# jsnchon/acai-omr

Measured on AMD Instinct MI355X. Metric: LMX tokens/sec (greedy decode, KV cache), higher is better.
Workload: dtype bf16; 1 GPU; vitomr_greedy_decode batch 8/GPU of 512x2048 images (4096 patches), decode steps 6..136; batch_per_gpu=8, memory_len=4096, decoder=12 x d1024 h16 mlp4096, V=227, hipgraph=True, split_merge=in-launch

## Files before the change

### acai_omr_amd/_lib.py

```python
import ctypes
import os
import subprocess
from ctypes import POINTER, Structure, c_char_p, c_double, c_float, c_int, c_int32, c_int64, c_uint32, c_void_p, c_size_t

CSRC = os.path.join(os.path.dirname(os.path.abspath(__file__)), "csrc")
LIB_PATH = os.environ.get("ACAI_OMR_LIB") or os.path.join(CSRC, "libacai_omr_hip.so")
SOURCES = ["gemm.hip", "gemm_tile.hip", "gemm_ring.hip", "gemm_pp.hip", "elementwise.hip", "attn.hip", "attn_varlen.hip", "attn_probs.hip", "confidence.hip", "attn_fwd64.hip", "attn_fwd64w.hip", "attn_bwd.hip", "attn_bwd64w.hip", "attn_bwd1p.hip", "train.hip", "grpo.hip", "seqdist.hip", "seqalign.hip", "grammar.hip", "decode.hip", "decode_gemv.hip", "decode_attn.hip", "decode_select.hip", "decode_prefill.hip", "resize.hip", "augment.hip", "page.hip", "deskew.hip", "flatten.hip", "rectify.hip", "ingest.hip", "prune.hip", "assess.hip"]

ACAI_F32, ACAI_BF16, ACAI_FP8_E4M3 = 0, 1, 2
GEMM_GELU, GEMM_ROUND_BF16 = 1, 2
(GEMM_K_REG, GEMM_K_GLDS, GEMM_K_GLDS3, GEMM_K_PERS, GEMM_K_256, GEMM_K_PERS256, GEMM_K_PP, GEMM_K_TN_GLDS, GEMM_K_TN_RING,
 GEMM_K_TN_PP) = range(10)
GEMM_KERNEL_NAMES = ("gemm_nt_kernel", "gemm_nt_glds_kernel", "gemm_nt_glds3_kernel", "gemm_nt_pers_kernel", "gemm_nt_256_kernel",
                     "gemm_nt_pers256_kernel", "gemm_nt_pp_kernel", "gemm_tn_glds_kernel", "gemm_tn_ring_kernel", "gemm_tn_pp_kernel")
GEMM_PP_OBF, GEMM_PP_GELU, GEMM_PP_AUX1, GEMM_PP_AUX2, GEMM_PP_RES, GEMM_PP_SCALE, GEMM_PP_DEFER, GEMM_PP_AUX3, GEMM_PP_AUX4 = 1, 2, 4, 8, 16, 32, 64, 128, 256
DEC_CROSS_FP8 = 256


class AcaiDecLayer(Structure):
    _fields_ = [(n, c_void_p) for n in (
        "self_in_w", "self_in_b", "self_out_w", "self_out_b", "cross_q_w", "cross_q_b", "cross_out_w", "cross_out_b",
        "lin1_w", "lin1_b", "lin2_w", "lin2_b", "n1_w", "n1_b", "n2_w", "n2_b", "n3_w", "n3_b",
        "k_self", "v_self", "k_cross", "v_cross", "k_cross_scale", "v_cross_scale")]

# ... 177 lines not shown
    "acai_page_warp": (c_int, [c_void_p, c_int, c_int, c_int, c_int, POINTER(c_int64), c_float, c_void_p, c_int, c_int, c_int, c_void_p]),
    "acai_page_ingest": (c_int, [c_void_p, c_int, c_int, c_int, c_int, c_int64, c_int64, c_int64, c_int, c_void_p, c_int, c_void_p]),
    "acai_page_col_profile": (c_int, [c_void_p, c_int, c_int, c_int, c_int, c_float, c_void_p, c_void_p, c_void_p, c_int64, c_void_p]),
    "acai_page_box_ink": (c_int, [c_void_p, c_int, c_int, c_int, c_int, c_float, c_void_p, c_int, c_void_p, c_void_p]),
    "acai_page_runs": (c_int, [c_void_p, c_int, c_int, c_int, c_int, c_float, c_void_p, c_void_p, c_int64, c_void_p]),
    "acai_page_sharpness": (c_int, [c_void_p, c_int, c_int, c_int, c_int, c_void_p, c_void_p]),
    "acai_patch_ink": (c_int, [c_void_p, c_int, c_int, c_int, c_int64, c_float, c_void_p, c_void_p]),
    "acai_patch_keep": (c_int, [c_void_p, c_void_p, c_int, c_int, c_int, c_int, c_void_p, c_void_p, c_void_p]),
    "acai_patch_compact": (c_int, [c_void_p, c_int, c_int, c_int64, c_void_p, c_void_p, c_void_p, c_int, c_int, c_void_p, c_void_p, c_void_p, c_void_p]),
    "acai_attn_map_expand": (c_int, [c_void_p, c_void_p, c_void_p, c_void_p, c_void_p, c_void_p, c_void_p, c_void_p, c_int, c_int, c_int, c_void_p]),
    "acai_gather_rows": (c_int, [c_void_p, c_void_p, c_void_p, c_void_p, c_int, c_int, c_void_p]),
    "acai_attn_varlen_fwd": (c_int, [c_void_p, c_int, c_void_p, c_int, c_void_p, c_int, c_void_p, c_int, c_void_p, c_void_p,
                                     c_int, c_int, c_int, c_int, c_int, c_int, c_void_p, c_int, c_float, c_uint32, c_int, c_void_p]),
    "acai_attn_probs_mean": (c_int, [c_void_p, c_int, c_void_p, c_int, c_void_p, c_void_p, c_int, c_int, c_int, c_int, c_int, c_int, c_void_p, c_int,
                                     c_void_p, c_void_p, c_void_p, c_int, c_void_p]),
    "acai_attn_map_locate": (c_int, [c_void_p, c_void_p, c_void_p, c_void_p, POINTER(c_int32), c_int, c_int, c_void_p, c_void_p, c_void_p]),
    "acai_token_confidence": (c_int, [c_void_p, c_void_p, c_int, c_int, c_int, c_float, c_void_p, c_void_p, c_void_p, c_void_p, c_void_p, c_void_p]),
    "acai_attn_map_weighted_sum": (c_int, [c_void_p, c_void_p, c_void_p, c_void_p, c_void_p, c_int, c_int, c_int, c_int64, c_void_p, c_void_p,
                                           c_void_p]),
    "acai_attn_varlen_bwd": (c_int, [c_void_p, c_int, c_void_p, c_int, c_void_p, c_int, c_void_p, c_int, c_void_p, c_int, c_void_p, c_int,
                                     c_void_p, c_int, c_void_p, c_int, c_void_p, c_void_p, c_void_p, c_void_p, c_int, c_int, c_int, c_int, c_int,
                                     c_int, c_int, c_int, c_float, c_uint32, c_int, c_void_p]),
    "acai_attn_varlen_bwd_ws": (c_int, [c_void_p, c_int, c_void_p, c_int, c_void_p, c_int, c_void_p, c_int, c_void_p, c_int, c_void_p, c_int,
                                        c_void_p, c_int, c_void_p, c_int, c_void_p, c_void_p, c_void_p, c_void_p, c_int, c_int, c_int, c_int, c_int,
                                        c_int, c_int, c_int, c_int, c_float, c_uint32, c_int, c_void_p, c_size_t, c_void_p]),
    "acai_attn_varlen_bwd_workspace_bytes": (c_size_t, [c_int, c_int, c_int, c_int, c_int, c_int, c_int, c_int, c_int, c_float, c_int]),
    "acai_attn_plan": (c_int, [POINTER(AcaiAttnQuery), POINTER(AcaiAttnLaunch), POINTER(c_int), POINTER(c_int)]),
    "acai_attn_last_plan": (c_int, [POINTER(AcaiAttnLaunch), POINTER(c_int)]),
    "acai_attn_set_override": (c_int, [c_int, c_int]),
    "acai_attn_get_override": (c_int, [c_int, POINTER(c_int)]),
    "acai_dropout_add": (c_int, [c_void_p, c_void_p, c_void_p, c_int, c_int, c_float, c_uint32, c_int, c_int, c_void_p]),
    "acai_layernorm_bwd": (c_int, [c_void_p, c_void_p, c_void_p, c_float, c_void_p, c_void_p, c_void_p, c_void_p, c_void_p, c_void_p, c_int, c_int, c_void_p]),
    "acai_gelu_fwd": (c_int, [c_void_p, c_void_p, c_int64, c_int, c_void_p]),
    "acai_gelu_bwd": (c_int, [c_void_p, c_void_p, c_void_p, c_int64, c_int, c_void_p]),
    "acai_adamw_step": (c_int, [c_void_p, c_void_p, c_void_p, c_void_p, c_int, c_int, c_float, c_void_p]),
    "acai_grad_norm": (c_int, [c_void_p, c_void_p, c_void_p, c_void_p, c_int, c_int, c_int, c_float, c_float, c_void_p, c_void_p, c_void_p, c_void_p]),
    "acai_adamw_step_clipped": (c_int, [c_void_p, c_void_p, c_void_p, c_void_p, c_int, c_int, c_float, c_void_p, c_int, c_void_p, c_void_p]),
    "acai_cast_weights": (c_int, [c_void_p, c_int, c_int, c_void_p]),
    "acai_gemm_dw": (c_int, [c_void_p, c_int, c_void_p, c_int, c_void_p, c_int, c_void_p, c_int, c_int, c_int, c_int, c_void_p]),
    "acai_colsum": (c_int, [c_void_p, c_int, c_void_p, c_int, c_int, c_int, c_void_p]),
    "acai_scatter_add_rows": (c_int, [c_void_p, c_void_p, c_void_p, c_int, c_int, c_int, c_void_p]),
    "acai_mae_loss": (c_int, [c_void_p, c_void_p, c_void_p, c_float, c_void_p, c_void_p, c_int, c_int, c_void_p]),
    "acai_ce_loss": (c_int, [c_void_p, c_int, c_void_p, c_int, c_float, c_float, c_void_p, c_void_p, c_int, c_int, c_void_p]),
    "acai_grpo_objective_fwd": (c_int, [c_void_p, c_int, c_void_p, c_int, c_void_p, c_int, c_void_p, c_void_p, c_int, c_int, c_int, c_float, c_float,
                                        c_int, c_float, c_void_p, c_void_p, c_void_p, c_void_p]),
    "acai_grpo_objective_bwd": (c_int, [c_void_p, c_int, c_void_p, c_int, c_void_p, c_void_p, c_void_p, c_void_p, c_int, c_int, c_int, c_int, c_float,
                                        c_void_p, c_void_p]),
    "acai_edit_distance": (c_int, [c_void_p, c_int, c_void_p, c_void_p, c_int, c_void_p, c_int, c_int, c_void_p, c_void_p]),
    "acai_edit_align_workspace_bytes": (c_size_t, [c_int, c_int, c_int]),
    "acai_edit_align": (c_int, [c_void_p, c_int, c_void_p, c_void_p, c_int, c_void_p, c_int, c_int, c_void_p, c_void_p, c_void_p, c_void_p, c_void_p,
                                c_void_p, c_size_t, c_void_p]),
    "acai_debug_stamps": (c_int, [c_void_p, c_int]),
    "acai_debug_lds_dma_oob": (c_int, [c_void_p, c_int, c_void_p, c_void_p]),
    "acai_pe_interp_fwd": (c_int, [c_void_p, c_int, c_int, c_int, c_void_p, c_int, c_int, c_void_p]),
    "acai_pe_interp_bwd": (c_int, [c_void_p, c_int, c_int, c_int, c_void_p, c_int, c_int, c_void_p]),
    "acai_cast_f32_bf16": (c_int, [c_void_p, c_void_p, c_int64, c_void_p]),
    "acai_skinny_gemm": (c_int, [c_void_p, c_int, c_void_p, c_int, c_void_p, c_void_p, c_int, c_void_p, c_int, c_int, c_int, c_int,
                                 c_int, c_int, c_void_p]),
    "acai_skinny_gemm_ex": (c_int, [c_void_p, c_int, c_int, c_void_p, c_int, c_void_p, c_void_p, c_int, c_void_p, c_int, c_int, c_int, c_int,
                                    c_int, c_int, c_int, c_void_p, c_void_p, c_float, c_void_p, c_void_p, c_void_p, c_void_p, c_void_p]),
    "acai_decode_attn": (c_int, [c_void_p, c_int, c_void_p, c_void_p, c_void_p, c_void_p, c_void_p, c_void_p, c_int, c_int, c_int,
                                 c_int, c_int, c_int, c_int, c_int, c_int, c_void_p, c_void_p]),
    "acai_decode_attn_fp8": (c_int, [c_void_p, c_int, c_void_p, c_void_p, c_void_p, c_void_p, c_void_p, c_void_p, c_void_p, c_void_p, c_int,
                                     c_int, c_int, c_int, c_int, c_int, c_int, c_int, c_void_p, c_void_p]),
    "acai_cross_kv_quantize_fp8": (c_int, [c_void_p, c_void_p, c_void_p, c_void_p, c_void_p, c_void_p, c_int64, c_int64, c_int, c_void_p]),
    "acai_decode_embed": (c_int, [POINTER(AcaiDecoder), c_void_p]),
    "acai_decode_step": (c_int, [POINTER(AcaiDecoder), c_void_p]),
    "acai_decode_sample_step": (c_int, [POINTER(AcaiDecoder), c_void_p, c_int, c_float, c_void_p]),
    "acai_decode_beam_step": (c_int, [POINTER(AcaiDecoder), POINTER(AcaiBeam), c_void_p]),
    "acai_decode_slot_step": (c_int, [POINTER(AcaiDecoder), POINTER(AcaiSlots), c_void_p]),
    "acai_decode_slot_sample_step": (c_int, [POINTER(AcaiDecoder), POINTER(AcaiSlots), c_void_p, c_int, c_void_p, c_int, c_float,
                                             c_void_p]),
    "acai_decode_slot_arm": (c_int, [POINTER(AcaiDecoder), POINTER(AcaiSlots), c_void_p, c_int, c_void_p]),
    "acai_decode_spec_arm": (c_int, [POINTER(AcaiDecoder), POINTER(AcaiSpec), c_void_p]),
    "acai_decode_spec_step": (c_int, [POINTER(AcaiDecoder), POINTER(AcaiSpec), c_void_p]),
    "acai_decode_prompt_step": (c_int, [POINTER(AcaiDecoder), POINTER(AcaiPrompt), c_void_p]),
    "acai_decode_spec_prompt_arm": (c_int, [POINTER(AcaiDecoder), POINTER(AcaiSpec), POINTER(AcaiPrompt), c_void_p]),
    "acai_decode_spec_prompt_step": (c_int, [POINTER(AcaiDecoder), POINTER(AcaiSpec), POINTER(AcaiPrompt), c_void_p]),
    "acai_decode_prefill_self_kv": (c_int, [POINTER(AcaiDecoder), c_int, c_void_p, c_int, c_int, c_void_p]),
    "acai_decode_prefill_arm": (c_int, [POINTER(AcaiDecoder), POINTER(AcaiPrompt), c_void_p, c_int, c_void_p]),
    "acai_decode_grammar_step": (c_int, [POINTER(AcaiDecoder), POINTER(AcaiGrammar), c_void_p]),
    "acai_decode_grammar_sample_step": (c_int, [POINTER(AcaiDecoder), POINTER(AcaiGrammar), c_void_p, c_int, c_float, c_void_p]),
    "acai_decode_slot_grammar_step": (c_int, [POINTER(AcaiDecoder), POINTER(AcaiSlots), POINTER(AcaiGrammar), c_void_p]),
    "acai_decode_slot_grammar_sample_step": (c_int, [POINTER(AcaiDecoder), POINTER(AcaiSlots), POINTER(AcaiGrammar), c_void_p, c_int, c_void_p,
                                                     c_int, c_float, c_void_p]),
    "acai_grammar_scan": (c_int, [c_void_p, c_int, c_void_p, c_int, c_void_p, c_void_p, c_int, c_int, c_int, c_int, c_void_p, c_void_p,
                                  c_void_p]),
    "acai_decode_logits": (c_int, [POINTER(AcaiDecoder), c_void_p, c_int, c_void_p]),
    "acai_decode_hidden": (c_int, [POINTER(AcaiDecoder), c_void_p, c_void_p]),
    "acai_decode_merge_in_launch": (c_int, [c_int, c_int]),
    "acai_graph_begin": (c_int, [c_void_p]),
    "acai_graph_end": (c_int, [c_void_p, POINTER(c_void_p)]),
    "acai_graph_launch": (c_int, [c_void_p, c_void_p]),
    "acai_graph_destroy": (c_int, [c_void_p]),
}

_lib = None


def build(force=False, verbose=False):
    from concurrent.futures import ThreadPoolExecutor
    srcs = [os.path.join(CSRC, s) for s in SOURCES if os.path.exists(os.path.join(CSRC, s))]
    hdrs = sorted(os.path.join(CSRC, f) for f in os.listdir(CSRC) if f.endswith(".h")) + [os.path.join(os.path.dirname(CSRC), "..", "include", "acai_omr_hip.h")]
    hipcc = "hipcc" if subprocess.run(["which", "hipcc"], capture_output=True).returncode == 0 else "/opt/rocm/bin/hipcc"
    flags = ["-O3", "--offload-arch=gfx950", "-std=c++17", "-fPIC", "-Wno-unused-value"]
    per_file = {"attn_varlen.hip": ["-fno-slp-vectorize"], "attn_fwd64.hip": ["-fno-slp-vectorize"],
# ... 79 lines not shown
```

### acai_omr_amd/csrc/common.h

```cpp
#pragma once
#include <hip/hip_runtime.h>
#include <stdint.h>
#include <stdio.h>
#include <string.h>

#include "../../include/acai_omr_hip.h"

typedef uint16_t bf16_t;
typedef __attribute__((ext_vector_type(8))) __bf16 bf16x8;
typedef __attribute__((ext_vector_type(2))) __bf16 bf16x2;
typedef __attribute__((ext_vector_type(16))) float f32x16;
typedef __attribute__((ext_vector_type(4))) float f32x4;

extern char g_acai_err[512];
int acai_set_err(int code, const char *fmt, ...);

#define ACAI_CHECK_ARG(cond, ...)                       \
    do {                                                \
        if (!(cond)) return acai_set_err(-1, __VA_ARGS__); \
    } while (0)

#define ACAI_LAUNCH_CHECK(name)                                                        \
    do {                                                                               \
        hipError_t e_ = hipGetLastError();                                             \
        if (e_ != hipSuccess) return acai_set_err((int)e_, "%s: %s", name, hipGetErrorString(e_)); \
    } while (0)

__device__ __forceinline__ float bf2f(bf16_t v) { return __uint_as_float(((uint32_t)v) << 16); }
__device__ __forceinline__ bf16_t f2bf(float f) {
    __bf16 h = (__bf16)f;
    return __builtin_bit_cast(bf16_t, h);
}
__device__ __forceinline__ float round_bf16(float f) { return bf2f(f2bf(f)); }
typedef __attribute__((ext_vector_type(2))) float f32x2;
__device__ __forceinline__ uint32_t pack_bf16(float lo, float hi) {
    const f32x2 v = {lo, hi};
    return __builtin_bit_cast(uint32_t, __builtin_convertvector(v, bf16x2));
}

__device__ __forceinline__ float fast_exp2(float x) { return __builtin_amdgcn_exp2f(x); }

__device__ __forceinline__ uint32_t drop_hash(uint32_t seed, uint32_t row, uint32_t col) {
    uint32_t x = (row * 0x9E3779B1u) ^ (col * 0x85EBCA77u) ^ seed;
    x ^= x >> 15; x *= 0x2C1B3C6Du;
    x ^= x >> 12; x *= 0x297A2D39u;
    x ^= x >> 15;
    return x;
}
__device__ __forceinline__ bool drop_keep(uint32_t seed, uint32_t row, uint32_t col, uint32_t thr) { return drop_hash(seed, row, col) >= thr; }

__device__ __forceinline__ uint4 ld_nt16(const void *p) {
    typedef __attribute__((ext_vector_type(4))) unsigned int u32x4;
    const u32x4 v = __builtin_nontemporal_load(reinterpret_cast<const u32x4 *>(p));
    return make_uint4(v[0], v[1], v[2], v[3]);
}

template <int ES, int DHP>
struct TileLayout {
    static constexpr int PITCH = ES == 2 ? DHP * 2 : DHP * 4 + 16;
    __device__ static __forceinline__ int swz(int row) {
        if constexpr (ES != 2) return 0;
        else if constexpr (DHP == 32) return (row >> 2) & 3;
        else return (((row >> 1) & 1) << 2) | ((row >> 2) & 3);
    }
    __device__ static __forceinline__ int off(int row, int chunk) { return row * PITCH + ((chunk ^ swz(row)) << 4); }
};

__device__ __forceinline__ float acai_half_erfc_abs(float x) {
    const float t = __builtin_amdgcn_fmed3f(fabsf(x) * 0.70710678118654752440f, 0.0f, 12.0f);
    float q = 1.420412202e-04f;
    q = fmaf(q, t, -3.664269981e-03f);
    q = fmaf(q, t, 3.089617088e-02f);
    q = fmaf(q, t, -1.496994187e-01f);
    q = fmaf(q, t, -9.181654744e-01f);
    q = fmaf(q, t, -1.627925070e+00f);
    return __builtin_amdgcn_exp2f(fmaf(q, t, -1.0f));
}

__device__ __forceinline__ float gelu_erf(float x) {
    return fmaf(-fabsf(x), acai_half_erfc_abs(x), __int_as_float(max(__float_as_int(x), 0)));
}

__device__ __forceinline__ float gelu_erf_grad(float x) {
    const float h = acai_half_erfc_abs(x);
    const float phi = x < 0.0f ? h : 1.0f - h;
    return fmaf(x, __builtin_amdgcn_exp2f(fmaf(x * x, -0.72134752044448170368f, -1.3257480647361593f)), phi);
}

__device__ __forceinline__ void gelu_erf_both(float x, float &g, float &dg) {
    const float h = acai_half_erfc_abs(x);
    g = fmaf(-fabsf(x), h, __int_as_float(max(__float_as_int(x), 0)));
    const float phi = x < 0.0f ? h : 1.0f - h;
    dg = fmaf(x, __builtin_amdgcn_exp2f(fmaf(x * x, -0.72134752044448170368f, -1.3257480647361593f)), phi);
}

template <typename T> struct DT;
template <> struct DT<float> {
    static constexpr int id = ACAI_F32;
    __device__ static __forceinline__ float ld(const float *p) { return *p; }
    __device__ static __forceinline__ void st(float *p, float v) { *p = v; }
};
template <> struct DT<bf16_t> {
    static constexpr int id = ACAI_BF16;
    __device__ static __forceinline__ float ld(const bf16_t *p) { return bf2f(*p); }
    __device__ static __forceinline__ void st(bf16_t *p, float v) { *p = f2bf(v); }
};

__device__ __forceinline__ float wave_sum_dpp(float v) {
#define ACAI_DPP_ADD(CTRL, ROWMASK) v += __builtin_bit_cast(float, __builtin_amdgcn_update_dpp(0, __builtin_bit_cast(int, v), CTRL, ROWMASK, 0xF, false))
    ACAI_DPP_ADD(0xB1, 0xF);
    ACAI_DPP_ADD(0x4E, 0xF);
    ACAI_DPP_ADD(0x141, 0xF);
    ACAI_DPP_ADD(0x140, 0xF);
    ACAI_DPP_ADD(0x142, 0xA);
    ACAI_DPP_ADD(0x143, 0xC);
#undef ACAI_DPP_ADD
    return __builtin_bit_cast(float, __builtin_amdgcn_readlane(__builtin_bit_cast(int, v), 63));
}

__device__ __forceinline__ float wave_sum(float v) {
#pragma unroll
    for (int o = 32; o > 0; o >>= 1) v += __shfl_xor(v, o);
    return v;
}
__device__ __forceinline__ float wave_max(float v) {
#pragma unroll
    for (int o = 32; o > 0; o >>= 1) v = fmaxf(v, __shfl_xor(v, o));
    return v;
}

__device__ __forceinline__ float row_argmax_sumexp(const float *lg, int V, int lane, float &best, int &bi) {
    best = -INFINITY;
    bi = 0x7fffffff;
    for (int i = lane; i < V; i += 64) {
        const float v = lg[i];
        if (v > best) {
            best = v;
            bi = i;
        }
    }
#pragma unroll
    for (int o = 32; o > 0; o >>= 1) {
        const float ov = __shfl_xor(best, o);
        const int oi = __shfl_xor(bi, o);
        if (ov > best || (ov == best && oi < bi)) {
            best = ov;
            bi = oi;
        }
    }
    float se = 0.f;
    for (int i = lane; i < V; i += 64) se += expf(lg[i] - best);
    return wave_sum(se);
}

__device__ __forceinline__ int prompt_len(const int32_t *plen, int row, int ppitch, int max_len) {
    return min(max(plen[row], 0), min(ppitch, max_len) - 1);
}

__device__ __forceinline__ int prompt_token(const int32_t *ptok, int row, int ppitch, int p, int len, int V) {
    if (p < 1 || p > len) return -1;
    const int v = ptok[(size_t)row * ppitch + p];
    return (v >= 0 && v < V) ? v : -1;
}

static inline int cdiv(int a, int b) { return (a + b - 1) / b; }
constexpr int ACAI_MAX_DEV = 64;
static inline bool acai_first_on_device(bool (&seen)[ACAI_MAX_DEV]) {
    int d = 0;
    if (hipGetDevice(&d) != hipSuccess || d < 0 || d >= ACAI_MAX_DEV) return true;
    if (seen[d]) return false;
    seen[d] = true;
// ... 4 lines not shown
```

### acai_omr_amd/csrc/decode_attn.hip

```cpp
#include "decode_internal.h"

namespace {

template <typename TC, int LPK, bool RAGGED, int U = 2, bool ANC = false, bool SLOT = false, bool SPEC = false>
__global__ __launch_bounds__(256) void decode_attn_kernel(DAttnArgs a) {
    static_assert(!(ANC && RAGGED), "the ancestor table indexes the self-attention cache");
    static_assert(!(SLOT && (RAGGED || ANC)), "the ring indexes the self-attention cache of the row itself");
    static_assert(!(SPEC && (RAGGED || ANC || SLOT)), "the key table indexes the self-attention cache of the image's rows");
    constexpr bool F8 = sizeof(TC) == 1;
    static_assert(!F8 || RAGGED, "FP8 storage is the cross K/V's only");
    constexpr int EPC = 16 / sizeof(TC), KPW = 64 / LPK;
    __shared__ float red[4][2 + 64];
    const int tid = threadIdx.x, lane = tid & 63, wave = tid >> 6;
    const int kq = lane % LPK, kg = lane / LPK;
    const int split = blockIdx.x, h = blockIdx.y, b = blockIdx.z;
    int len, hstride;
    size_t base;
    if constexpr (RAGGED) {
        len = a.seq_len[b];
        hstride = len * a.dhp;
        base = (size_t)a.seq_off[b] + (size_t)h * hstride;
    } else if constexpr (ANC) {
        len = a.step[1] + 1;
        hstride = a.Tmax * a.dhp;
        base = (size_t)h * hstride;
    } else if constexpr (SLOT) {
        len = a.seq_len[b];
        hstride = a.Tmax * a.dhp;
        base = ((size_t)b * a.H + h) * hstride;
    } else if constexpr (SPEC) {
        const int R = (int)a.anc_bstride, img = b / R;
        len = max(1, min(a.seq_len[img] + (b - img * R), min(a.anc_pitch, a.chunk * a.nsplit)));
        hstride = a.Tmax * a.dhp;
        base = ((size_t)img * R * a.H + h) * hstride;
    } else {
        len = a.step[1] + 1;
        hstride = a.Tmax * a.dhp;
        base = ((size_t)b * a.H + h) * hstride;
    }
    float *part = a.partial + (((size_t)b * a.H + h) * a.nsplit + split) * (a.dhp + 2);
    const int c0 = split * a.chunk, c1 = min(len, c0 + a.chunk);
    const bool fused_merge = a.tickets && a.out && a.nsplit > 1;
    if (c0 >= len) {
        if (tid < a.dhp + 2) {
            if (fused_merge) __hip_atomic_store(part + tid, tid == 0 ? -1.0e30f : 0.f, __ATOMIC_RELAXED, __HIP_MEMORY_SCOPE_AGENT);
            else part[tid] = tid == 0 ? -1.0e30f : 0.f;
        }
        if (!fused_merge) return;
        asm volatile("s_waitcnt vmcnt(0)" ::: "memory");
    }
    const TC *Kp = reinterpret_cast<const TC *>(a.kc) + base;
    const TC *Vp = reinterpret_cast<const TC *>(a.vc) + base;
    [[maybe_unused]] const float *Ks = nullptr, *Vs = nullptr;
    if constexpr (F8) {
        const size_t row0 = base >> __builtin_ctz(a.dhp);
        Ks = a.k_scale + row0;
        Vs = a.v_scale + row0;
    }
    [[maybe_unused]] int32_t *anc_s = nullptr;
    if constexpr (ANC) {
        extern __shared__ int32_t anc_dyn[];
        anc_s = anc_dyn;
        const int32_t *ar = a.anc + (size_t)(a.step[0] & 1) * a.anc_bstride + (size_t)b * a.anc_pitch;
        for (int p = c0 + tid; p < c1; p += 256) anc_s[p - c0] = ar[p];
        __syncthreads();
    }
    if constexpr (SPEC) {
        extern __shared__ int32_t anc_dyn[];
        anc_s = anc_dyn;
        const int32_t *tr = a.spec_tab + (size_t)(b / (int)a.anc_bstride) * a.anc_pitch;
        for (int p = c0 + tid; p < c1; p += 256) anc_s[p - c0] = tr[p];
        __syncthreads();
    }
    [[maybe_unused]] int ring0 = 0;
    if constexpr (SLOT) ring0 = a.slot_first[b];
    auto key_off = [&](int key) -> size_t {
        if constexpr (ANC) return (size_t)anc_s[key - c0] * a.H * hstride + (size_t)key * a.dhp;
        else if constexpr (SPEC) {
            const unsigned e = (unsigned)anc_s[key - c0];
            const int r = min((int)(e & 7u), (int)a.anc_bstride - 1), pos = min((int)(e >> 3), a.Tmax - 1);
            return (size_t)r * a.H * hstride + (size_t)pos * a.dhp;
        }
        else if constexpr (SLOT) {
            const int p = ring0 + key;
            return (size_t)(p >= a.Tmax ? p - a.Tmax : p) * a.dhp;
        } else return (size_t)key * a.dhp;
    };

    float qf[EPC];
#pragma unroll
    for (int e = 0; e < EPC; ++e) {
        const int d = kq * EPC + e;
        qf[e] = d < a.dh ? a.q[(size_t)b * a.ldq + h * a.dh + d] : 0.f;
    }
    float m = -1.0e30f, l = 0.f, acc[EPC];
#pragma unroll
    for (int e = 0; e < EPC; ++e) acc[e] = 0.f;

    uint4 kn[U], vn[U];
    [[maybe_unused]] float ksn[U], vsn[U];
    auto request = [&](int key0) {
#pragma unroll
        for (int u = 0; u < U; ++u) {
            const int key = key0 + u * 4 * KPW;
            kn[u] = vn[u] = make_uint4(0, 0, 0, 0);
            if constexpr (F8) ksn[u] = vsn[u] = 0.f;
            if (key < c1) {
                kn[u] = ld_nt16(Kp + key_off(key) + kq * EPC);
                vn[u] = ld_nt16(Vp + key_off(key) + kq * EPC);
                if constexpr (F8) {
                    ksn[u] = __builtin_nontemporal_load(Ks + key);
                    vsn[u] = __builtin_nontemporal_load(Vs + key);
                }
            }
        }
    };
    request(c0 + wave * KPW + kg);
    for (int key0 = c0 + wave * KPW + kg; key0 < c1; key0 += 4 * KPW * U) {
        uint4 kk[U], vv[U];
        [[maybe_unused]] float ks[U], vs[U];
#pragma unroll
        for (int u = 0; u < U; ++u) {
            kk[u] = kn[u];
            vv[u] = vn[u];
            if constexpr (F8) {
                ks[u] = ksn[u];
                vs[u] = vsn[u];
            }
        }
        if (key0 + 4 * KPW * U < c1) request(key0 + 4 * KPW * U);
#pragma unroll
        for (int u = 0; u < U; ++u) {
            const int key = key0 + u * 4 * KPW;
            float kf[EPC], vf[EPC];
            if constexpr (F8) {
                const uint32_t kw[4] = {kk[u].x, kk[u].y, kk[u].z, kk[u].w}, vw[4] = {vv[u].x, vv[u].y, vv[u].z, vv[u].w};
#pragma unroll
                for (int e = 0; e < 4; ++e) {
                    const auto k0 = __builtin_amdgcn_cvt_pk_f32_fp8((int)kw[e], false), k1 = __builtin_amdgcn_cvt_pk_f32_fp8((int)kw[e], true);
                    const auto v0 = __builtin_amdgcn_cvt_pk_f32_fp8((int)vw[e], false), v1 = __builtin_amdgcn_cvt_pk_f32_fp8((int)vw[e], true);
                    kf[4 * e] = k0[0];
                    kf[4 * e + 1] = k0[1];
                    kf[4 * e + 2] = k1[0];
                    kf[4 * e + 3] = k1[1];
                    vf[4 * e] = v0[0];
                    vf[4 * e + 1] = v0[1];
                    vf[4 * e + 2] = v1[0];
                    vf[4 * e + 3] = v1[1];
                }
            } else if constexpr (sizeof(TC) == 2) {
                const uint32_t kw[4] = {kk[u].x, kk[u].y, kk[u].z, kk[u].w}, vw[4] = {vv[u].x, vv[u].y, vv[u].z, vv[u].w};
#pragma unroll
                for (int e = 0; e < 4; ++e) {
                    kf[2 * e] = __uint_as_float(kw[e] << 16);
                    kf[2 * e + 1] = __uint_as_float(kw[e] & 0xffff0000u);
                    vf[2 * e] = __uint_as_float(vw[e] << 16);
                    vf[2 * e + 1] = __uint_as_float(vw[e] & 0xffff0000u);
                }
            } else {
                const f32x4 k4 = __builtin_bit_cast(f32x4, kk[u]), v4 = __builtin_bit_cast(f32x4, vv[u]);
#pragma unroll
                for (int e = 0; e < 4; ++e) {
                    kf[e] = k4[e];
                    vf[e] = v4[e];
                }
            }
            float s = 0.f;
#pragma unroll
            for (int e = 0; e < EPC; ++e) s = fmaf(qf[e], kf[e], s);
#pragma unroll
            for (int o = 1; o < LPK; o <<= 1) s += __shfl_xor(s, o);
            if (key < c1) {
                if constexpr (F8) s *= ks[u];
                s *= a.scale_log2e;
                const float mn = fmaxf(m, s), al = fast_exp2(m - mn), p = fast_exp2(s - mn);
                m = mn;
                l = l * al + p;
                float pv = p;
                if constexpr (F8) pv *= vs[u];
#pragma unroll
                for (int e = 0; e < EPC; ++e) acc[e] = acc[e] * al + pv * vf[e];
            }
        }
    }
    float mw = m;
#pragma unroll
    for (int o = LPK; o < 64; o <<= 1) mw = fmaxf(mw, __shfl_xor(mw, o));
    const float f = fast_exp2(m - mw);
    l *= f;
#pragma unroll
    for (int e = 0; e < EPC; ++e) acc[e] *= f;
#pragma unroll
    for (int o = LPK; o < 64; o <<= 1) {
        l += __shfl_xor(l, o);
#pragma unroll
        for (int e = 0; e < EPC; ++e) acc[e] += __shfl_xor(acc[e], o);
    }
    if (kg == 0) {
        if (kq == 0) {
            red[wave][0] = mw;
            red[wave][1] = l;
        }
#pragma unroll
        for (int e = 0; e < EPC; ++e) red[wave][2 + kq * EPC + e] = acc[e];
    }
    __syncthreads();
    if (wave != 0) return;
    const int d = lane;
    const float M = fmaxf(fmaxf(red[0][0], red[1][0]), fmaxf(red[2][0], red[3][0]));
    float v = 0.f, lsum = 0.f;
#pragma unroll
    for (int w = 0; w < 4; ++w) {
        const float f = fast_exp2(red[w][0] - M);
        v += red[w][2 + d] * f;
        lsum += red[w][1] * f;
    }
    if (a.nsplit == 1 && a.out) {
        if (d < a.dh) {
            float o = v / lsum;
            if (a.round_out) o = round_bf16(o);
            if (a.out_bf16) reinterpret_cast<bf16_t *>(a.out)[(size_t)b * a.ldo + h * a.dh + d] = f2bf(o);
            else a.out[(size_t)b * a.ldo + h * a.dh + d] = o;
        }
        return;
    }
    if (c0 < len && d < a.dhp) {
        if (fused_merge) {
            __hip_atomic_store(part + 2 + d, v, __ATOMIC_RELAXED, __HIP_MEMORY_SCOPE_AGENT);
            if (d == 0) {
                __hip_atomic_store(part, M, __ATOMIC_RELAXED, __HIP_MEMORY_SCOPE_AGENT);
                __hip_atomic_store(part + 1, lsum, __ATOMIC_RELAXED, __HIP_MEMORY_SCOPE_AGENT);
            }
        } else {
            part[2 + d] = v;
            if (d == 0) {
                part[0] = M;
                part[1] = lsum;
            }
        }
    }
    if (!fused_merge) return;
    asm volatile("s_waitcnt vmcnt(0)" ::: "memory");
    int last = 0;
    if (lane == 0) {
        unsigned *cnt = a.tickets + (size_t)b * a.H + h;
        const unsigned t = __hip_atomic_fetch_add(cnt, 1u, __ATOMIC_RELAXED, __HIP_MEMORY_SCOPE_AGENT);
        last = t == (unsigned)(a.nsplit - 1);
        if (last) __hip_atomic_store(cnt, 0u, __ATOMIC_RELAXED, __HIP_MEMORY_SCOPE_AGENT);
    }
    last = __builtin_amdgcn_readfirstlane(last);
// ... 178 lines not shown
    }
    if (fused_merge) {
        __shared__ int s_last;
        asm volatile("s_waitcnt vmcnt(0)" ::: "memory");
        __syncthreads();
        if (tid == 0) {
            unsigned *cnt = a.tickets + (size_t)row0 * a.H + h;
            const unsigned t = __hip_atomic_fetch_add(cnt, 1u, __ATOMIC_RELAXED, __HIP_MEMORY_SCOPE_AGENT);
            const int last = t == (unsigned)(a.nsplit - 1);
            if (last) __hip_atomic_store(cnt, 0u, __ATOMIC_RELAXED, __HIP_MEMORY_SCOPE_AGENT);
            s_last = last;
        }
        __syncthreads();
        if (s_last) {
            const int d = tid & 63;
            for (int g = tid >> 6; g < ng; g += 4) {
                float *pp = a.partial + ((size_t)(row0 + g) * a.H + h) * a.nsplit * (DHP + 2);
                auto ld = [&](int i) { return __hip_atomic_load(pp + i, __ATOMIC_RELAXED, __HIP_MEMORY_SCOPE_AGENT); };
                float M = -1.0e30f, ls = 0.f, o = 0.f;
                for (int s0 = 0; s0 < a.nsplit; s0 += 8) {
                    float pm[8], pl[8], po[8];
#pragma unroll
                    for (int u = 0; u < 8; ++u) {
                        const bool in = s0 + u < a.nsplit;
                        const int base = (in ? s0 + u : s0) * (DHP + 2);
                        pm[u] = in ? ld(base) : -1.0e30f;
                        pl[u] = in ? ld(base + 1) : 0.f;
                        po[u] = in ? ld(base + 2 + d) : 0.f;
                    }
                    float Mc = M;
#pragma unroll
                    for (int u = 0; u < 8; ++u) Mc = fmaxf(Mc, pm[u]);
                    const float resc = fast_exp2(M - Mc);
                    ls *= resc;
                    o *= resc;
                    M = Mc;
#pragma unroll
                    for (int u = 0; u < 8; ++u) {
                        const float w = fast_exp2(pm[u] - M);
                        ls += pl[u] * w;
                        o += po[u] * w;
                    }
                }
                if (d < a.dh) {
                    float v = o / ls;
                    if (a.round_out) v = round_bf16(v);
                    a.out[(size_t)(row0 + g) * a.ldo + h * a.dh + d] = v;
                }
            }
        }
    }
}

__global__ __launch_bounds__(64) void attn_combine_kernel(const float *partial, float *out, int ldo, int H, int dh, int dhp,
                                                          int nsplit, int round_out) {
    const int h = blockIdx.x, b = blockIdx.y, d = threadIdx.x;
    const float *p = partial + ((size_t)b * H + h) * nsplit * (dhp + 2);
    float M = -1.0e30f;
    for (int s = 0; s < nsplit; ++s) M = fmaxf(M, p[s * (dhp + 2)]);
    float l = 0.f, o = 0.f;
    for (int s = 0; s < nsplit; ++s) {
        const float w = fast_exp2(p[s * (dhp + 2)] - M);
        l += p[s * (dhp + 2) + 1] * w;
        if (d < dhp) o += p[s * (dhp + 2) + 2 + d] * w;
    }
    if (d < dh) {
        float v = o / l;
        if (round_out) v = round_bf16(v);
        out[(size_t)b * ldo + h * dh + d] = v;
    }
}

__device__ __forceinline__ float pow2i(int e) { return __int_as_float((e + 127) << 23); }

template <int LPR>
__device__ __forceinline__ void quantize_row_part(const bf16_t *in, uint8_t *out, float *scale, int part) {
    const uint4 w0 = *reinterpret_cast<const uint4 *>(in), w1 = *reinterpret_cast<const uint4 *>(in + 8);
    const uint32_t w[8] = {w0.x, w0.y, w0.z, w0.w, w1.x, w1.y, w1.z, w1.w};
    float x[16], amax = 0.f;
#pragma unroll
    for (int i = 0; i < 8; ++i) {
        x[2 * i] = __uint_as_float(w[i] << 16);
        x[2 * i + 1] = __uint_as_float(w[i] & 0xffff0000u);
        amax = fmaxf(amax, fmaxf(fabsf(x[2 * i]), fabsf(x[2 * i + 1])));
    }
#pragma unroll
    for (int o = 1; o < LPR; o <<= 1) amax = fmaxf(amax, __shfl_xor(amax, o));
    int k = 0;
    const float m = frexpf(amax, &k);
    const int e = amax > 0.f ? max(k - 9 + (m > 0.875f ? 1 : 0), -126) : 0;
    const float inv = pow2i(-e);
    uint32_t q[4];
#pragma unroll
    for (int i = 0; i < 4; ++i) {
        int v = __builtin_amdgcn_cvt_pk_fp8_f32(x[4 * i] * inv, x[4 * i + 1] * inv, 0, false);
        v = __builtin_amdgcn_cvt_pk_fp8_f32(x[4 * i + 2] * inv, x[4 * i + 3] * inv, v, true);
        q[i] = (uint32_t)v;
    }
    *reinterpret_cast<uint4 *>(out) = make_uint4(q[0], q[1], q[2], q[3]);
    if (part == 0) *scale = pow2i(e);
}

template <int LPR>
__global__ __launch_bounds__(256) void cross_kv_quantize_fp8_kernel(const bf16_t *kin, const bf16_t *vin, uint8_t *k8, uint8_t *v8, float *ks,
                                                                    float *vs, long long row0, long long nrows) {
    constexpr int DHP = 16 * LPR;
// ... 100 lines not shown
    if (nrows == 0) return 0;
    const int lpr = dhp / 16;
    const dim3 grid((unsigned)((nrows * lpr + 255) / 256));
    hipStream_t st = (hipStream_t)stream;
    auto kin = (const bf16_t *)k_in, vin = (const bf16_t *)v_in;
    auto k8 = (uint8_t *)k_out, v8 = (uint8_t *)v_out;
    if (lpr == 1) hipLaunchKernelGGL(cross_kv_quantize_fp8_kernel<1>, grid, dim3(256), 0, st, kin, vin, k8, v8, k_scale, v_scale, (long long)row0, (long long)nrows);
    else if (lpr == 2) hipLaunchKernelGGL(cross_kv_quantize_fp8_kernel<2>, grid, dim3(256), 0, st, kin, vin, k8, v8, k_scale, v_scale, (long long)row0, (long long)nrows);
    else hipLaunchKernelGGL(cross_kv_quantize_fp8_kernel<4>, grid, dim3(256), 0, st, kin, vin, k8, v8, k_scale, v_scale, (long long)row0, (long long)nrows);
    ACAI_LAUNCH_CHECK("cross_kv_quantize_fp8");
    return 0;
}

extern "C" int acai_decode_attn(const float *q, int ldq, const void *kc, const void *vc, const int64_t *seq_off, const int32_t *seq_len,
                                float *partial, float *out, int ldo, int B, int H, int dh, int dhp, int chunk, int nsplit, int dtype,
                                int round_out, uint32_t *tickets, void *stream) {
    ACAI_CHECK_ARG(q && kc && vc && seq_off && seq_len && partial, "acai_decode_attn: null operand");
    ACAI_CHECK_ARG(B > 0 && H > 0 && dh > 0 && dhp >= dh && dhp <= 64 && (dhp & (dhp - 1)) == 0 && chunk > 0 && nsplit > 0,
                   "acai_decode_attn: bad dims");
    DAttnArgs a{};
    a.q = q; a.kc = kc; a.vc = vc; a.seq_off = seq_off; a.seq_len = seq_len; a.partial = partial;
    a.ldq = ldq; a.H = H; a.dh = dh; a.dhp = dhp; a.chunk = chunk; a.nsplit = nsplit;
    a.scale_log2e = 1.4426950408889634f / sqrtf((float)dh);
    hipStream_t st = (hipStream_t)stream;
    if (tickets && out) {
        a.out = out; a.ldo = ldo; a.round_out = round_out; a.tickets = tickets;
        return dtype == ACAI_BF16 ? launch_dattn<bf16_t>(a, B, false, st) : launch_dattn<float>(a, B, false, st);
    }
    int rc = dtype == ACAI_BF16 ? launch_dattn<bf16_t>(a, B, false, st) : launch_dattn<float>(a, B, false, st);
    if (rc || !out) return rc;
    return launch_attn_combine(partial, out, ldo, B, H, dh, dhp, nsplit, round_out, st);
}

extern "C" int acai_decode_attn_fp8(const float *q, int ldq, const void *kc, const void *vc, const float *k_scale, const float *v_scale,
                                    const int64_t *seq_off, const int32_t *seq_len, float *partial, float *out, int ldo, int B, int H, int dh,
                                    int dhp, int chunk, int nsplit, int round_out, uint32_t *tickets, void *stream) {
    ACAI_CHECK_ARG(q && kc && vc && k_scale && v_scale && seq_off && seq_len && partial, "acai_decode_attn_fp8: null operand");
    ACAI_CHECK_ARG(B > 0 && H > 0 && dh > 0 && dhp >= dh && (dhp == 16 || dhp == 32 || dhp == 64) && chunk > 0 && nsplit > 0,
                   "acai_decode_attn_fp8: bad dims");
    DAttnArgs a{};
    a.q = q; a.kc = kc; a.vc = vc; a.k_scale = k_scale; a.v_scale = v_scale; a.seq_off = seq_off; a.seq_len = seq_len; a.partial = partial;
    a.ldq = ldq; a.H = H; a.dh = dh; a.dhp = dhp; a.chunk = chunk; a.nsplit = nsplit;
    a.scale_log2e = 1.4426950408889634f / sqrtf((float)dh);
    hipStream_t st = (hipStream_t)stream;
    if (tickets && out) {
        a.out = out; a.ldo = ldo; a.round_out = round_out; a.tickets = tickets;
        return launch_dattn_fp8(a, B, st);
    }
    int rc = launch_dattn_fp8(a, B, st);
    if (rc || !out) return rc;
    return launch_attn_combine(partial, out, ldo, B, H, dh, dhp, nsplit, round_out, st);
}

extern "C" int acai_decode_merge_in_launch(int dtype, int dhp) {
    if (dtype == ACAI_FP8_E4M3)
        ACAI_CHECK_ARG(dhp == 16 || dhp == 32 || dhp == 64, "acai_decode_merge_in_launch: bad FP8 dhp");
    else
        ACAI_CHECK_ARG((dtype == ACAI_BF16 || dtype == ACAI_F32) && dhp > 0 && dhp <= 64 && (dhp & (dhp - 1)) == 0, "acai_decode_merge_in_launch: bad dtype / dhp");
    return dattn_merge_in_launch(dtype, dhp) ? 1 : 0;
}
```

### include/acai_omr_hip.h

```cpp
#ifndef ACAI_OMR_HIP_H
#define ACAI_OMR_HIP_H

#include <stdint.h>

#ifdef __cplusplus
extern "C" {
#endif

#define ACAI_ABI_VERSION 1
#define ACAI_F32 0
#define ACAI_BF16 1
#define ACAI_FP8_E4M3 2

#define ACAI_GEMM_GELU 1
#define ACAI_GEMM_ROUND_BF16 2

int acai_version(void);
const char *acai_last_error(void);

int acai_layernorm_fwd(const float *x, const float *w, const float *b, float eps, float *out_f32, void *out_bf16,
                       int rows, int dim, void *stream);

int acai_gemm_nt(const void *A, int lda, const void *W, int ldw, const float *bias, const float *residual, int ldr,
                 void *C, int ldc, int M, int N, int K, int in_dtype, int out_dtype, int flags, void *stream);
// ... 15 lines not shown
    ACAI_GEMM_K_GLDS = 1,
    ACAI_GEMM_K_GLDS3 = 2,
    ACAI_GEMM_K_PERS = 3,
    ACAI_GEMM_K_256 = 4,
    ACAI_GEMM_K_PERS256 = 5,
    ACAI_GEMM_K_PP = 6,
    ACAI_GEMM_K_TN_GLDS = 7,
    ACAI_GEMM_K_TN_RING = 8,
    ACAI_GEMM_K_TN_PP = 9
};
enum { ACAI_PP_OBF = 1, ACAI_PP_GELU = 2, ACAI_PP_AUX1 = 4, ACAI_PP_AUX2 = 8, ACAI_PP_RES = 16, ACAI_PP_SCALE = 32,
       ACAI_PP_DEFER = 64, ACAI_PP_AUX3 = 128, ACAI_PP_AUX4 = 256 };
typedef struct AcaiGemmQuery {
    int elem_size;
    int epi;
    int trans_a, trans_w;
    int M, N, K;
    int lda, ldw, ldc, ldr, ldaux;
    int a_aligned, w_aligned, c_aligned, r_aligned, aux_aligned;
    int out_dtype, flags, aux_mode;
    int has_residual;
    int scale_cols;
    int want_colsum;
    int variant;
    int n_cu;
} AcaiGemmQuery;
typedef struct AcaiGemmLaunch {
    int kernel;
    int wm, fast, pp_mode;
    int grid, block;
    int ksplit, vec_epi;
    int row0, rows;
    int k0, k;
    int colsum;
} AcaiGemmLaunch;
int acai_gemm_plan(const AcaiGemmQuery *query, AcaiGemmLaunch *launches_out, int *n_out);
int acai_gemm_last_plan(AcaiGemmLaunch *launches_out, int *n_out);

int acai_patchify(const float *img, int H, int W, int P, void *out, int ld, int row0, int out_dtype, void *stream);

int acai_resize_bicubic_aa(const float *img, int C, int H, int W, float *tmp, float *out, int OH, int OW, int clamp01, void *stream);

int acai_resize_to_patches(const void *img, int in_u8, int H, int W, float *tmp, void *patches, int ld, int row0, int OH, int OW, int top,
                           int left, int ch, int cw, int P, int out_dtype, int clamp01, void *stream);

int acai_gather_rows(const float *table, const int32_t *idx, const float *add, float *out, int rows, int dim, void *stream);

int acai_pe_interp_fwd(const float *table, int Hin, int Win, int E, float *out, int Hout, int Wout, void *stream);
int acai_pe_interp_bwd(const float *dout, int Hout, int Wout, int E, float *dtable, int Hin, int Win, void *stream);

int acai_debug_stamps(void *buf, int cap_launches);

int acai_debug_lds_dma_oob(const void *src, int valid_bytes, void *out, void *stream);

int acai_cast_f32_bf16(const float *x, void *y, int64_t n, void *stream);

int acai_attn_varlen_fwd(const void *q, int ldq, const void *k, int ldk, const void *v, int ldv, void *out, int ldo,
                         const int32_t *cu_q, const int32_t *cu_k, int B, int H, int dh, int max_q, int causal,
                         int dtype, float *lse, int total_q, float dropout_p, uint32_t dropout_seed, int q_prescaled, void *stream);

int acai_attn_varlen_bwd(const void *q, int ldq, const void *k, int ldk, const void *v, int ldv, const void *o, int ldo,
                         const void *dout, int lddo, void *dq, int lddq, void *dk, int lddk, void *dv, int lddv, const float *lse,
                         float *delta, const int32_t *cu_q, const int32_t *cu_k, int B, int H, int dh, int max_q, int max_k,
                         int total_q, int causal, int dtype, float dropout_p, uint32_t dropout_seed, int q_prescaled, void *stream);
size_t acai_attn_varlen_bwd_workspace_bytes(int B, int H, int dh, int max_q, int max_k, int total_q, int total_k, int causal, int dtype,
                                            float dropout_p, int q_prescaled);
int acai_attn_varlen_bwd_ws(const void *q, int ldq, const void *k, int ldk, const void *v, int ldv, const void *o, int ldo,
                            const void *dout, int lddo, void *dq, int lddq, void *dk, int lddk, void *dv, int lddv, const float *lse,
                            float *delta, const int32_t *cu_q, const int32_t *cu_k, int B, int H, int dh, int max_q, int max_k,
                            int total_q, int total_k, int causal, int dtype, float dropout_p, uint32_t dropout_seed, int q_prescaled,
                            void *workspace, size_t workspace_bytes, void *stream);

enum {
    ACAI_ATTN_K_FWD = 0,
    ACAI_ATTN_K_FWD64 = 1,
    ACAI_ATTN_K_FWD64W = 2,
    ACAI_ATTN_K_FWD64_TAIL = 3,
    ACAI_ATTN_K_BWD_DQ = 4,
    ACAI_ATTN_K_BWD_DKV = 5,
    ACAI_ATTN_K_BWD_DQ2 = 6,
    ACAI_ATTN_K_BWD_DKV2 = 7,
    ACAI_ATTN_K_BWD64W_DQ = 8,
    ACAI_ATTN_K_BWD64W_DKV = 9,
    ACAI_ATTN_K_BWD1P = 10
};
enum {
    ACAI_ATTN_OV_TWO_BLOCK = 0,
    ACAI_ATTN_OV_FWD64 = 1,
    ACAI_ATTN_OV_BWD64_WIDE = 2,
    ACAI_ATTN_OV_BWD_1P = 3,
    ACAI_ATTN_OV_XCD_ORDER = 4,
    ACAI_ATTN_OV_COUNT = 5
};
enum { ACAI_ATTN_FWD64_AUTO = 0 , ACAI_ATTN_FWD64_NW4 = 1, ACAI_ATTN_FWD64_NW8 = 2 ,
       ACAI_ATTN_FWD64_GENERIC = 3  };
enum { ACAI_ATTN_REFUSE_NONE = 0, ACAI_ATTN_REFUSE_PRESCALED = 1 ,
       ACAI_ATTN_REFUSE_ACCUM = 2  };
typedef struct AcaiAttnQuery {
    int backward;
    int elem_size;
    int B, H, dh, max_q, max_k, total_q, total_k;
    int causal, accum_dkv, dropout, q_prescaled;
    int ldq, ldk, ldv, ldo, lddo, lddq, lddk, lddv;
    int aligned;
    int cu_k_is_cu_q;
    int ov[ACAI_ATTN_OV_COUNT];
// ... 341 lines not shown
```

Measured before the change: 11820 tokens/s.

## Prefetch first KV tile and q early, use DPP/permlane butterflies in decode attention

In the plain (non-ragged, non-slot) decode attention path, the step length is read through the scalar constant address space. The q vector and the first K/V tile are issued before the index setup, so global-load latency overlaps the prologue. The shuffle-based dot-product reductions and cross-lane softmax merges are replaced with DPP and permlane16/32 swap butterflies, which avoid LDS-backed ds_bpermute. A debug probe kernel is added to check the new lane-xor helpers against __shfl_xor. The risks are extra register pressure from holding the prefetched tiles and correctness depending on the DPP encodings.

```diff
diff --git a/acai_omr_amd/_lib.py b/acai_omr_amd/_lib.py
--- a/acai_omr_amd/_lib.py
+++ b/acai_omr_amd/_lib.py
@@ -253,6 +253,7 @@
                                 c_void_p, c_size_t, c_void_p]),
     "acai_debug_stamps": (c_int, [c_void_p, c_int]),
     "acai_debug_lds_dma_oob": (c_int, [c_void_p, c_int, c_void_p, c_void_p]),
+    "acai_debug_lane_xor": (c_int, [c_void_p, c_int, c_int, c_int, c_void_p, c_void_p]),
     "acai_pe_interp_fwd": (c_int, [c_void_p, c_int, c_int, c_int, c_void_p, c_int, c_int, c_void_p]),
     "acai_pe_interp_bwd": (c_int, [c_void_p, c_int, c_int, c_int, c_void_p, c_int, c_int, c_void_p]),
     "acai_cast_f32_bf16": (c_int, [c_void_p, c_void_p, c_int64, c_void_p]),
diff --git a/acai_omr_amd/csrc/common.h b/acai_omr_amd/csrc/common.h
--- a/acai_omr_amd/csrc/common.h
+++ b/acai_omr_amd/csrc/common.h
@@ -53,6 +53,11 @@
     typedef __attribute__((ext_vector_type(4))) unsigned int u32x4;
     const u32x4 v = __builtin_nontemporal_load(reinterpret_cast<const u32x4 *>(p));
     return make_uint4(v[0], v[1], v[2], v[3]);
+}
+
+template <typename T>
+__device__ __forceinline__ T ld_uniform(const T *p) {
+    return *reinterpret_cast<const __attribute__((address_space(4))) T *>(reinterpret_cast<uintptr_t>(p));
 }
 
 template <int ES, int DHP>
@@ -117,6 +122,29 @@
 #undef ACAI_DPP_ADD
     return __builtin_bit_cast(float, __builtin_amdgcn_readlane(__builtin_bit_cast(int, v), 63));
 }
+
+template <int O>
+__device__ __forceinline__ float lane_xor(float v) {
+    static_assert(O == 1 || O == 2 || O == 4 || O == 8 || O == 16 || O == 32, "one butterfly stage of a wave of 64");
+    const int x = __builtin_bit_cast(int, v);
+    if constexpr (O == 1) return __builtin_bit_cast(float, __builtin_amdgcn_update_dpp(0, x, 0xB1, 0xF, 0xF, false));
+    else if constexpr (O == 2) return __builtin_bit_cast(float, __builtin_amdgcn_update_dpp(0, x, 0x4E, 0xF, 0xF, false));
+    else if constexpr (O == 8) return __builtin_bit_cast(float, __builtin_amdgcn_update_dpp(0, x, 0x128, 0xF, 0xF, false));
+    else if constexpr (O == 16) {
+        const auto r = __builtin_amdgcn_permlane16_swap((unsigned)x, (unsigned)x, false, false);
+        return __builtin_bit_cast(float, (__lane_id() & 16) ? r[0] : r[1]);
+    } else if constexpr (O == 32) {
+        const auto r = __builtin_amdgcn_permlane32_swap((unsigned)x, (unsigned)x, false, false);
+        return __builtin_bit_cast(float, (__lane_id() & 32) ? r[0] : r[1]);
+    } else return __shfl_xor(v, O);
+}
+__device__ __forceinline__ float lane_xor4_quad_uniform(float v) {
+    return __builtin_bit_cast(float, __builtin_amdgcn_update_dpp(0, __builtin_bit_cast(int, v), 0x141, 0xF, 0xF, false));
+}
+template <int O>
+__device__ __forceinline__ float lane_xor_add(float v) { return v + lane_xor<O>(v); }
+template <int O>
+__device__ __forceinline__ float lane_xor_max(float v) { return fmaxf(v, lane_xor<O>(v)); }
 
 __device__ __forceinline__ float wave_sum(float v) {
 #pragma unroll
diff --git a/acai_omr_amd/csrc/decode_attn.hip b/acai_omr_amd/csrc/decode_attn.hip
--- a/acai_omr_amd/csrc/decode_attn.hip
+++ b/acai_omr_amd/csrc/decode_attn.hip
@@ -14,12 +14,61 @@
     const int tid = threadIdx.x, lane = tid & 63, wave = tid >> 6;
     const int kq = lane % LPK, kg = lane / LPK;
     const int split = blockIdx.x, h = blockIdx.y, b = blockIdx.z;
+    constexpr bool PLAIN = !RAGGED && !ANC && !SLOT && !SPEC;
+    asm volatile("" ::"s"(a.q), "s"(a.kc), "s"(a.vc), "s"(a.partial), "s"(a.ldq), "s"(a.H), "s"(a.dh), "s"(a.dhp), "s"(a.Tmax), "s"(a.chunk),
+                 "s"(a.nsplit), "s"(a.scale_log2e), "s"(a.out), "s"(a.ldo), "s"(a.round_out), "s"(a.tickets), "s"(a.out_bf16));
+    if constexpr (RAGGED) asm volatile("" ::"s"(a.seq_off), "s"(a.seq_len));
+    if constexpr (PLAIN || ANC) asm volatile("" ::"s"(a.step));
+    if constexpr (SLOT || SPEC) asm volatile("" ::"s"(a.seq_len));
+    if constexpr (ANC || SLOT || SPEC) asm volatile("" ::"s"(a.anc), "s"(a.anc_pitch), "s"(a.anc_bstride));
+    if constexpr (F8) asm volatile("" ::"s"(a.k_scale), "s"(a.v_scale));
+    [[maybe_unused]] int len_raw = 0;
+    [[maybe_unused]] int64_t off_raw = 0;
+    if constexpr (RAGGED) {
+        len_raw = ld_uniform(a.seq_len + b);
+        off_raw = ld_uniform(a.seq_off + b);
+    } else if constexpr (PLAIN) len_raw = ld_uniform(a.step + 1);
+
+    float qf[EPC];
+    auto request_q = [&]() {
+        const float *qr = a.q + (size_t)b * a.ldq + h * a.dh;
+        if ((((uintptr_t)a.q | (uintptr_t)(unsigned)a.ldq * 4 | (uintptr_t)(unsigned)a.dh * 4) & 15) == 0 && a.dh >= 4) {
+#pragma unroll
+            for (int j = 0; j < EPC / 4; ++j) {
+                const f32x4 v = *reinterpret_cast<const f32x4 *>(qr + min(kq * EPC + 4 * j, a.dh - 4));
+#pragma unroll
+                for (int e = 0; e < 4; ++e) qf[4 * j + e] = v[e];
+            }
+        } else {
+#pragma unroll
+            for (int e = 0; e < EPC; ++e) qf[e] = qr[min(kq * EPC + e, a.dh - 1)];
+        }
+    };
+    auto zero_q_past_dh = [&]() {
+#pragma unroll
+        for (int e = 0; e < EPC; ++e) qf[e] = kq * EPC + e < a.dh ? qf[e] : 0.f;
+    };
+    if constexpr (!ANC && !SPEC) request_q();
+    uint4 kn[U], vn[U];
+    if constexpr (PLAIN) {
+        const TC *K0 = reinterpret_cast<const TC *>(a.kc) + ((size_t)b * a.H + h) * ((size_t)a.Tmax * a.dhp) + kq * EPC;
+        const TC *V0 = reinterpret_cast<const TC *>(a.vc) + ((size_t)b * a.H + h) * ((size_t)a.Tmax * a.dhp) + kq * EPC;
+#pragma unroll
+        for (int u = 0; u < U; ++u) {
+            const int key = max(min(split * a.chunk + wave * KPW + kg + u * 4 * KPW, a.Tmax - 1), 0);
+            kn[u] = ld_nt16(K0 + (size_t)key * a.dhp);
+            vn[u] = ld_nt16(V0 + (size_t)key * a.dhp);
+        }
+    }
+    __builtin_amdgcn_sched_barrier(0);
+    if constexpr (!ANC && !SPEC) zero_q_past_dh();
+
     int len, hstride;
     size_t base;
     if constexpr (RAGGED) {
-        len = a.seq_len[b];
+        len = len_raw;
         hstride = len * a.dhp;
-        base = (size_t)a.seq_off[b] + (size_t)h * hstride;
+        base = (size_t)off_raw + (size_t)h * hstride;
     } else if constexpr (ANC) {
         len = a.step[1] + 1;
         hstride = a.Tmax * a.dhp;
@@ -34,7 +83,7 @@
         hstride = a.Tmax * a.dhp;
         base = ((size_t)img * R * a.H + h) * hstride;
     } else {
-        len = a.step[1] + 1;
+        len = len_raw + 1;
         hstride = a.Tmax * a.dhp;
         base = ((size_t)b * a.H + h) * hstride;
     }
@@ -87,17 +136,14 @@
         } else return (size_t)key * a.dhp;
     };
 
-    float qf[EPC];
-#pragma unroll
-    for (int e = 0; e < EPC; ++e) {
-        const int d = kq * EPC + e;
-        qf[e] = d < a.dh ? a.q[(size_t)b * a.ldq + h * a.dh + d] : 0.f;
+    if constexpr (ANC || SPEC) {
+        request_q();
+        zero_q_past_dh();
     }
     float m = -1.0e30f, l = 0.f, acc[EPC];
 #pragma unroll
     for (int e = 0; e < EPC; ++e) acc[e] = 0.f;
 
-    uint4 kn[U], vn[U];
     [[maybe_unused]] float ksn[U], vsn[U];
     auto request = [&](int key0) {
 #pragma unroll
@@ -115,7 +161,7 @@
             }
         }
     };
-    request(c0 + wave * KPW + kg);
+    if constexpr (!PLAIN) request(c0 + wave * KPW + kg);
     for (int key0 = c0 + wave * KPW + kg; key0 < c1; key0 += 4 * KPW * U) {
         uint4 kk[U], vv[U];
         [[maybe_unused]] float ks[U], vs[U];
@@ -168,8 +214,10 @@
             float s = 0.f;
 #pragma unroll
             for (int e = 0; e < EPC; ++e) s = fmaf(qf[e], kf[e], s);
-#pragma unroll
-            for (int o = 1; o < LPK; o <<= 1) s += __shfl_xor(s, o);
+            if constexpr (LPK > 1) s = lane_xor_add<1>(s);
+            if constexpr (LPK > 2) s = lane_xor_add<2>(s);
+            if constexpr (LPK > 4) s += lane_xor4_quad_uniform(s);
+            if constexpr (LPK > 8) s = lane_xor_add<8>(s);
             if (key < c1) {
                 if constexpr (F8) s *= ks[u];
                 s *= a.scale_log2e;
@@ -184,18 +232,21 @@
         }
     }
     float mw = m;
-#pragma unroll
-    for (int o = LPK; o < 64; o <<= 1) mw = fmaxf(mw, __shfl_xor(mw, o));
+#define ACAI_MERGE_STAGE(O)                                  \
+    if constexpr (LPK <= O) mw = lane_xor_max<O>(mw);
+    ACAI_MERGE_STAGE(1) ACAI_MERGE_STAGE(2) ACAI_MERGE_STAGE(4) ACAI_MERGE_STAGE(8) ACAI_MERGE_STAGE(16) ACAI_MERGE_STAGE(32)
+#undef ACAI_MERGE_STAGE
     const float f = fast_exp2(m - mw);
     l *= f;
 #pragma unroll
     for (int e = 0; e < EPC; ++e) acc[e] *= f;
-#pragma unroll
-    for (int o = LPK; o < 64; o <<= 1) {
-        l += __shfl_xor(l, o);
-#pragma unroll
-        for (int e = 0; e < EPC; ++e) acc[e] += __shfl_xor(acc[e], o);
-    }
+#define ACAI_MERGE_STAGE(O)                                  \
+    if constexpr (LPK <= O) {                                \
+        l = lane_xor_add<O>(l);                              \
+        _Pragma("unroll") for (int e = 0; e < EPC; ++e) acc[e] = lane_xor_add<O>(acc[e]); \
+    }
+    ACAI_MERGE_STAGE(1) ACAI_MERGE_STAGE(2) ACAI_MERGE_STAGE(4) ACAI_MERGE_STAGE(8) ACAI_MERGE_STAGE(16) ACAI_MERGE_STAGE(32)
+#undef ACAI_MERGE_STAGE
     if (kg == 0) {
         if (kq == 0) {
             red[wave][0] = mw;
@@ -480,6 +531,17 @@
     }
 }
 
+template <int O, bool MAX>
+__global__ __launch_bounds__(64) void lane_xor_probe_kernel(const float *in, float *out, int rows) {
+    const int r = blockIdx.x, lane = threadIdx.x;
+    const float v = in[(size_t)r * 64 + lane], w = __shfl_xor(v, O);
+    float got;
+    if constexpr (O == 4) got = MAX ? fmaxf(v, lane_xor4_quad_uniform(v)) : v + lane_xor4_quad_uniform(v);
+    else got = MAX ? lane_xor_max<O>(v) : lane_xor_add<O>(v);
+    out[(size_t)r * 64 + lane] = got;
+    out[((size_t)rows + r) * 64 + lane] = MAX ? fmaxf(v, w) : v + w;
+}
+
 __global__ __launch_bounds__(64) void attn_combine_kernel(const float *partial, float *out, int ldo, int H, int dh, int dhp,
                                                           int nsplit, int round_out) {
     const int h = blockIdx.x, b = blockIdx.y, d = threadIdx.x;
@@ -686,6 +748,23 @@
     return launch_attn_combine(partial, out, ldo, B, H, dh, dhp, nsplit, round_out, st);
 }
 
+extern "C" int acai_debug_lane_xor(const float *in, int rows, int offset, int op, float *out, void *stream) {
+    ACAI_CHECK_ARG(in && out && rows > 0 && (op == 0 || op == 1), "acai_debug_lane_xor: bad arguments");
+    hipStream_t st = (hipStream_t)stream;
+#define ACAI_LX(O)                                                                                                  \
+    case O:                                                                                                         \
+        if (op) hipLaunchKernelGGL((lane_xor_probe_kernel<O, true>), dim3(rows), dim3(64), 0, st, in, out, rows);   \
+        else hipLaunchKernelGGL((lane_xor_probe_kernel<O, false>), dim3(rows), dim3(64), 0, st, in, out, rows);     \
+        break;
+    switch (offset) {
+        ACAI_LX(1) ACAI_LX(2) ACAI_LX(4) ACAI_LX(8) ACAI_LX(16) ACAI_LX(32)
+        default: return acai_set_err(-1, "acai_debug_lane_xor: offset %d is no butterfly stage of a wave of 64", offset);
+    }
+#undef ACAI_LX
+    ACAI_LAUNCH_CHECK("acai_debug_lane_xor");
+    return 0;
+}
+
 extern "C" int acai_decode_merge_in_launch(int dtype, int dhp) {
     if (dtype == ACAI_FP8_E4M3)
         ACAI_CHECK_ARG(dhp == 16 || dhp == 32 || dhp == 64, "acai_decode_merge_in_launch: bad FP8 dhp");
diff --git a/include/acai_omr_hip.h b/include/acai_omr_hip.h
--- a/include/acai_omr_hip.h
+++ b/include/acai_omr_hip.h
@@ -91,6 +91,8 @@
 int acai_debug_stamps(void *buf, int cap_launches);
 
 int acai_debug_lds_dma_oob(const void *src, int valid_bytes, void *out, void *stream);
+
+int acai_debug_lane_xor(const float *in, int rows, int offset, int op, float *out, void *stream);
 
 int acai_cast_f32_bf16(const float *x, void *y, int64_t n, void *stream);
 
```

Measured after the change: 11980 tokens/s, median of 6. +1.3%, better.
